# real-stanford/flingbot

Hardware: AMD Instinct MI355X
Metric: sim steps/sec (64x64-particle cloth) (higher is better)
Workload: dtype f32

## Files before the change

flingbot_amd/csrc/fs_fused_grid_kernel.h:

```cpp
#pragma once
#include "fs_fused_kernel.h"

#define FG_PLANE (FS_FUSED_MAX_PARTICLES * 4)
#define FG_PAD 1024
#define FG_OFF_XX FG_PAD
#define FG_OFF_X0 (FG_OFF_XX + 4 * FG_PLANE)
#define FG_OFF_CACC (FG_OFF_X0 + 3 * FG_PLANE)
#define FG_OFF_CUR (FG_OFF_CACC + FS_FUSED_CSET_CAP * 16)
#define FG_OFF_ITEMS (FG_OFF_CUR + FS_FUSED_CUR_BYTES)
#define FG_OFF_SCAN (FG_OFF_ITEMS + FS_FUSED_MAX_PARTICLES * 2)
#define FG_OFF_CSET (FG_OFF_SCAN + 64)
#define FG_OFF_CHIST (FG_OFF_CSET + FS_FUSED_CSET_CAP * 2)
#define FG_OFF_ROWL (FG_OFF_CHIST + 512)
#define FG_OFF_KZ (FG_OFF_ROWL + 1024)
#define FG_OFF_KS (FG_OFF_KZ + 1024)
#define FG_OFF_COLL (FG_OFF_KS + 1024)
#define FG_OFF_RCNT (FG_OFF_COLL + 512)
#define FG_LDS_BYTES (FG_OFF_RCNT + 512)
static_assert(FG_OFF_ROWL % 8 == 0 && (FG_OFF_KZ - FG_OFF_ROWL) % 8 == 0, "row tables are read as ds_read_b64 pairs");
static_assert((FG_OFF_COLL - FG_OFF_KS) % 256 == 0, "column tables share one address, rows as ds_read2st64_b32 offsets");
static_assert(FG_LDS_BYTES <= 160 * 1024, "grid-64 kernel: the LDS of one CU");
static_assert(FG_OFF_CACC % 16 == 0 && FG_OFF_CUR == FG_OFF_CACC + FS_FUSED_CSET_CAP * 16, "set and queue accumulators: one array");
#ifndef FG_SINGLES
#define FG_SINGLES 1
// ... 74 lines not shown
    unsigned short *items = (unsigned short *)(smem + FG_OFF_ITEMS);
    int *wave_tot = (int *)(smem + FG_OFF_SCAN);
    float *rowL = (float *)(smem + FG_OFF_ROWL);

#ifdef FS_BLOCK_CLOCKS
    const unsigned long long tc_start = __builtin_amdgcn_s_memtime(), tr_start = __builtin_amdgcn_s_memrealtime();
#endif
#ifdef FS_TIMING
    unsigned long long ts_acc[16] = {0, 0, 0, 0, 0, 0, 0, 0, 0, 0, 0, 0, 0, 0, 0, 0};
    unsigned long long ts_last = __builtin_amdgcn_s_memtime();
#endif
    const int e = ids[blockIdx.x];
    if (e < 0) return;
    const FsEnvDev &E = envs[e];
    const FsShapesDev &sh = shapes[e];
    const FsFusedConsts c = fs_fused_consts(E, sh);
    const int n = c.n;
    const unsigned un = (unsigned)n;
    const int t = threadIdx.x, lane = t & 63, w = t >> 6;
    const int dimz = n >> 6;

    FsVec4 *const g_pos = E.pos;
    const FsVec4 *const g_rest = E.rest;
    const fs_gci g_phase = (fs_gci)E.phase;
    const fs_gi g_nlist = (fs_gi)E.nlist, g_ncount = (fs_gi)E.ncount;
    const fs_gci g_ell_j = (fs_gci)E.ell_j;
    const fs_gcf g_ell_len = (fs_gcf)E.ell_len, g_ell_k = (fs_gcf)E.ell_k;
    const fs_gcf g_L = (fs_gcf)E.g64_L;
    const int max_deg = E.max_deg;
    const fs_gcu g_near = (fs_gcu)E.restnear_w;

    int find_mode = 0;
    {
        const int ph0 = g_phase[0];
        int differs = 0;
        for (int i = t; i < n; i += FS_FUSED_THREADS) differs |= (g_phase[i] != ph0);
        if (t == 0) wave_tot[0] = 0;
        __syncthreads();
        if (differs) atomicOr(&wave_tot[0], 1);
        __syncthreads();
        const int mixed = wave_tot[0];
        __syncthreads();
        if (!mixed) {
            if (!(ph0 & FS_PHASE_SELF_COLLIDE)) find_mode = 3;
            else if (!(ph0 & FS_PHASE_SELF_COLLIDE_FILTER)) find_mode = 2;
            else if (E.restnear_ok == 2 && FS_STENCIL_FILTER) find_mode = 4;
            else if (E.restnear_ok) find_mode = 1;
        }
    }
    for (int q = t; q < FG_OFF_X0 / 4; q += FS_FUSED_THREADS) ((float *)smem)[q] = 0.0f;
    __syncthreads();
    for (int i = t; i < n; i += FS_FUSED_THREADS) {
        const FsVec4 p = fs_ld4(g_pos, i);
        Xx[i] = p.x; Xy[i] = p.y; Xz[i] = p.z; Xw[i] = p.w;
        X0x[i] = p.x; X0y[i] = p.y; X0z[i] = p.z;
    }
    if (t < 256) {
        const int r = t & 63, s = 8 + (t >> 6);
        rowL[t] = r < dimz ? g_L[(unsigned)s * un + (unsigned)(r * 64 + 2)] : 0.0f;
    }
    constexpr int XS_DX[4] = {-1, -2, +1, +2};
    constexpr int SH_DX[4] = {+1, -1, -1, +1}, SH_DZ[4] = {-1, -1, +1, +1};
    constexpr int ZS_DZ[4] = {-1, -2, +1, +2};
    float *colL = (float *)(smem + FG_OFF_COLL);
    if (t < 128) {
        const int col = t & 63, q = t >> 6;
        const int dxq = q == 0 ? -1 : -2;
        colL[t] = (unsigned)(col + dxq) < 64u ? g_L[(unsigned)q * un + (unsigned)(2 * 64 + col)] : 0.0f;
    }
    float *rcnt = (float *)(smem + FG_OFF_RCNT);
    if (t < 128) rcnt[t] = t > 0 ? c.relax / (float)t : 0.0f;
    if (t < 256) {
        const int c64 = t & 63, q = t >> 6;
        const int sdx = (q == 0 || q == 3) ? +1 : -1, sslot = q < 2 ? 2 + q : 4 + q;
        const int zdz = q < 2 ? -1 - q : q - 1;
        ((float *)(smem + FG_OFF_KS))[t] = (unsigned)(c64 + sdx) < 64u ? E.g64_kh[sslot] : 0.0f;
        ((float *)(smem + FG_OFF_KZ))[t] = (c64 < dimz && (unsigned)(c64 + zdz) < (unsigned)dimz) ? E.g64_kh[8 + q] : 0.0f;
    }
    const float kh0 = E.g64_kh[0], kh1 = E.g64_kh[1];
    unsigned nvalid = 0u;
#pragma unroll
    for (int k = 0; k < FS_FUSED_PPT; ++k) {
        const int row = FG_ROW(w, k);
        int cnt = 0;
#pragma unroll
        for (int q = 0; q < 4; ++q) {
            cnt += ((unsigned)(lane + XS_DX[q]) < 64u) ? 1 : 0;
            cnt += ((unsigned)(lane + SH_DX[q]) < 64u && (unsigned)(row + SH_DZ[q]) < (unsigned)dimz) ? 1 : 0;
            cnt += ((unsigned)(row + ZS_DZ[q]) < (unsigned)dimz) ? 1 : 0;
        }
        nvalid |= (unsigned)cnt << (8 * k);
    }
    __syncthreads();
    unsigned fastmask = 0u;
    {
        constexpr int cdx[FS_G64_SLOTS] = FS_G64_DX_LIST, cdz[FS_G64_SLOTS] = FS_G64_DZ_LIST;
#pragma unroll
        for (int k = 0; k < FS_FUSED_PPT; ++k) {
            const int row = FG_ROW(w, k), i = row * 64 + lane;
            bool differs = false;
            if (i < n) {
                const float wi = Xw[i];
                differs = !(wi > 0.0f);
#pragma unroll
                for (int q = 0; q < FS_G64_SLOTS; ++q) {
                    const bool in = (unsigned)(lane + cdx[q]) < 64u && (unsigned)(row + cdz[q]) < (unsigned)dimz;
                    if (in) differs |= Xw[i + cdz[q] * 64 + cdx[q]] != wi;
                }
            }
            if (i < n && __builtin_amdgcn_ballot_w64(differs) == 0ull) fastmask |= 1u << k;
        }
        fastmask = (unsigned)__builtin_amdgcn_readfirstlane((int)fastmask);
    }

    FsVec4 sx[FS_FUSED_PPT], sv[FS_FUSED_PPT];
#pragma unroll
    for (int k = 0; k < FS_FUSED_PPT; ++k) {
        const int i = t + k * FS_FUSED_THREADS;
        sx[k] = FsVec4{0.0f, 0.0f, 0.0f, 0.0f};
        sv[k] = FsVec4{0.0f, 0.0f, 0.0f, 0.0f};
        if (i < n) {
            sv[k] = fs_ld4o(E.vel, (unsigned)i);
            sx[k] = FsVec4{X0x[i], X0y[i], X0z[i], Xw[i]};
        }
    }

    FS_TS(0)
#pragma unroll 1
    for (int frame = 0; frame < n_steps; ++frame) {
#pragma unroll 1
        for (int sub = 0; sub < c.substeps; ++sub) {
            FsVec4 xp[FS_FUSED_PPT];
            {
                unsigned tl = (unsigned)t;
                asm volatile("" : "+v"(tl));
                for (unsigned q = tl; q < FS_FUSED_BUCKETS / 2; q += FS_FUSED_THREADS) ((unsigned *)cursor)[q] = 0u;
                FsFusedConsts cf = c;
                asm volatile("" : "+v"(cf.h), "+v"(cf.g0), "+v"(cf.g1), "+v"(cf.g2), "+v"(cf.damping));
#pragma unroll
                for (int k = 0; k < FS_FUSED_PPT; ++k) {
                    const unsigned i = tl + (unsigned)(k * FS_FUSED_THREADS);
                    xp[k] = FsVec4{0.0f, 0.0f, 0.0f, 0.0f};
                    if (i < un) xp[k] = fs_fused_predict(cf, sx[k], sv[k]);
                }
#pragma unroll
                for (int k = 0; k < FS_FUSED_PPT; ++k) {
                    const unsigned i = tl + (unsigned)(k * FS_FUSED_THREADS);
                    if (i < un) fs_st4o(E.x0, i, sx[k]);
                }
            }
            FS_TS(12)
            __syncthreads();
            const fs_lu fill = (fs_lu)(smem + FG_OFF_XX + 2 * FG_PLANE);
            if (find_mode == 4) {
                unsigned tl = (unsigned)t;
                asm volatile("" : "+v"(tl));
                for (unsigned q = tl; q < FS_FUSED_MAX_PARTICLES; q += FS_FUSED_THREADS) fill[q] = 0u;
            }
            unsigned xslot[2];
            {
                int slot_of[FS_FUSED_PPT] = {0, 0, 0, 0};
                fs_fused_build_grid(c, xp, cursor, items, wave_tot, X0x, X0y, X0z, slot_of);
                xslot[0] = (unsigned)slot_of[0] | ((unsigned)slot_of[1] << 16);
                xslot[1] = (unsigned)slot_of[2] | ((unsigned)slot_of[3] << 16);
            }
            FS_TS(1)
            const FsFindConsts fc = {n, c.ncap, c.rad2, c.inv_rad, find_mode, E.gp_dimx, E.gp_magic};
            if (find_mode == 4) {
                int *const any_over = wave_tot;
                if (t == 0) *any_over = 0;
                int sb0 = 0, sb1 = 0, sb2 = 0, sb3 = 0;
#pragma unroll 1
                for (int k = 0; k < FS_FUSED_PPT; ++k) {
                    const int qs = t + k * FS_FUSED_THREADS;
                    if (qs >= n) break;
                    const int i = items[qs];
                    const FsVec4 xi = FsVec4{X0x[qs], X0y[qs], X0z[qs], 0.0f};
                    const int shape_bits = (int)(fs_shape_candidates(E.p, sh, sub, xi.x, xi.y, xi.z) << FS_SHAPE_MASK_SHIFT);
                    if (k == 0) sb0 = shape_bits; else if (k == 1) sb1 = shape_bits; else if (k == 2) sb2 = shape_bits; else sb3 = shape_bits;
                    fs_pair_find_neighbors(fc, i, qs, xi, (fs_lcus)cursor, (fs_lcus)items, g_nlist, (fs_lus)(smem + FG_OFF_XX) + t,
                                           (fs_lcf)X0x, fill);
                }
                FS_TS(2)
                __syncthreads();
                FS_TS(3)
                unsigned overmask = 0u;
#pragma unroll 1
                for (int k = 0; k < FS_FUSED_PPT; ++k) {
                    const int qs = t + k * FS_FUSED_THREADS;
                    if (qs >= n) break;
                    const int i = items[qs];
                    const int cnt = (int)fill[i];
                    const int shape_bits = k == 0 ? sb0 : k == 1 ? sb1 : k == 2 ? sb2 : sb3;
                    if (cnt > c.ncap) {
                        overmask |= 1u << k;
                        continue;
                    }
                    fs_pair_sort_column(n, i, cnt, g_nlist);
                    g_ncount[i] = cnt | shape_bits;
                }
                if (overmask) atomicOr(any_over, 1);
                __syncthreads();
                if (*any_over) {
                    FsNearWords none;
#pragma unroll
                    for (int q = 0; q < 8; ++q) none.w[q] = 0xffffffffu;
#pragma unroll 1
                    for (int k = 0; k < FS_FUSED_PPT; ++k) {
                        if (!((overmask >> k) & 1u)) continue;
                        const int qs = t + k * FS_FUSED_THREADS;
                        const int i = items[qs];
                        const FsVec4 xi = FsVec4{X0x[qs], X0y[qs], X0z[qs], 0.0f};
                        const int shape_bits = k == 0 ? sb0 : k == 1 ? sb1 : k == 2 ? sb2 : sb3;
                        g_ncount[i] = fs_fused_find_neighbors<true>(fc, i, xi, (fs_lcus)cursor, (fs_lcus)items, g_phase, g_rest, g_nlist,
                                                                    none, (fs_lus)(smem + FG_OFF_XX) + t, (fs_lcf)X0x) | shape_bits;
                    }
                    __syncthreads();
                }
                FS_TS(15)
            } else {
#pragma unroll 1
                for (int qs = t; qs < n; qs += FS_FUSED_THREADS) {
                    const int i = items[qs];
                    const FsVec4 xi = FsVec4{X0x[qs], X0y[qs], X0z[qs], 0.0f};
                    const int shape_bits = (int)(fs_shape_candidates(E.p, sh, sub, xi.x, xi.y, xi.z) << FS_SHAPE_MASK_SHIFT);
                    FsNearWords near;
#pragma unroll
                    for (int q = 0; q < 8; ++q) near.w[q] = find_mode == 1 ? g_near[(unsigned)q * un + (unsigned)i] : 0xffffffffu;
                    g_ncount[i] = (find_mode == 3 ? 0
                                                  : fs_fused_find_neighbors<false>(fc, i, xi, (fs_lcus)cursor, (fs_lcus)items, g_phase,
                                                                                   g_rest, g_nlist, near,
                                                                                   (fs_lus)(smem + FG_OFF_XX) + t, (fs_lcf)X0x)) |
                                  shape_bits;
                }
                FS_TS(2)
                __syncthreads();
                FS_TS(3)
            }
            FsVec4 p0r[FS_FUSED_PPT];
            int cword[FS_FUSED_PPT];
            {
                unsigned tl = (unsigned)t;
                asm volatile("" : "+v"(tl));
#pragma unroll
                for (int k = 0; k < FS_FUSED_PPT; ++k) {
                    const unsigned i = tl + (unsigned)(k * FS_FUSED_THREADS);
                    p0r[k] = fs_ld4o(E.x0, i < un ? i : 0u);
                }
                const unsigned wl = tl >> 6, ll = tl & 63u;
#pragma unroll
                for (int k = 0; k < FS_FUSED_PPT; ++k) {
                    const unsigned i = (unsigned)FG_ROW(wl, k) * 64u + ll;
                    cword[k] = fs_ldo((const int *)E.ncount, i < un ? i : 0u);
                }
#pragma unroll
                for (int k = 0; k < FS_FUSED_PPT; ++k) {
                    const unsigned i = tl + (unsigned)(k * FS_FUSED_THREADS);
                    const unsigned s = (xslot[k >> 1] >> (16 * (k & 1))) & 0xffffu;
                    const float x = X0x[s], y = X0y[s], z = X0z[s];
                    if (i < un) {
                        Xx[i] = x; Xy[i] = y; Xz[i] = z; Xw[i] = p0r[k].w;
                    } else {
                        Xx[i] = 0.0f; Xy[i] = 0.0f; Xz[i] = 0.0f; Xw[i] = 0.0f;
                    }
                }
            }

            FS_TS(13)
            unsigned short *cset = (unsigned short *)(smem + FG_OFF_CSET);
            FsVec4 *cacc = (FsVec4 *)(smem + FG_OFF_CACC);
            int *chist = (int *)(smem + FG_OFF_CHIST);
            if (t < 128) chist[t] = 0;
            int *nsingles = (int *)(smem + FG_OFF_SCAN);
            if (t == 0) *nsingles = 0;
            __syncthreads();
            {
                unsigned tl = (unsigned)t;
                asm volatile("" : "+v"(tl));
#pragma unroll
                for (int k = 0; k < FS_FUSED_PPT; ++k) {
                    const unsigned i = tl + (unsigned)(k * FS_FUSED_THREADS);
                    if (i < un) { X0x[i] = p0r[k].x; X0y[i] = p0r[k].y; X0z[i] = p0r[k].z; }
                }
            }
            unsigned tq = (unsigned)t;
            asm volatile("" : "+v"(tq));
            const int wq = (int)(tq >> 6), lq = (int)(tq & 63u);
            int ccls[FS_FUSED_PPT];
#pragma unroll
            for (int k = 0; k < FS_FUSED_PPT; ++k) {
                const int i = FG_ROW(wq, k) * 64 + lq;
                int cc = 0;
                if (i < n && Xw[i] > 0.0f) cc = cword[k] & FS_NCOUNT_MASK;
                ccls[k] = cc > 96 ? 96 : cc;
                if (ccls[k] > 0) atomicAdd(&chist[ccls[k]], 1);
            }
            __syncthreads();
            fs_fused_count_offsets(chist, t);
            __syncthreads();
            FsVec4 *squeue = cacc + FS_FUSED_CSET_CAP;
            unsigned slotw[2] = {~0u, ~0u};
#pragma unroll
            for (int k = 0; k < FS_FUSED_PPT; ++k) {
                if (ccls[k] > 0) {
                    const int i = FG_ROW(wq, k) * 64 + lq;
                    unsigned slot = FG_SLOT_INLINE;
                    const int pos = atomicAdd(&chist[ccls[k]], 1);
                    if (pos < FS_FUSED_CSET_CAP) {
                        cset[pos] = (unsigned short)i;
                        slot = (unsigned)pos;
                    }
#if FG_SINGLES
                    else if (ccls[k] <= 16) {
                        const int sp = atomicAdd(nsingles, 1);
                        if (sp < FG_SINGLES_CAP) {
                            slot = (unsigned)(FS_FUSED_CSET_CAP + sp);
                            squeue[sp].w = __int_as_float(i | (fs_ldo((const int *)E.nlist, (unsigned)i) << 12) | ((ccls[k] - 1) << 28));
                        }
                    }
#endif
                    slotw[k >> 1] = (slotw[k >> 1] & ~(0xffffu << (16 * (k & 1)))) | (slot << (16 * (k & 1)));
                }
            }
            FS_TS(14)
            __syncthreads();
            const int csize = chist[0] < FS_FUSED_CSET_CAP ? chist[0] : FS_FUSED_CSET_CAP;
            const int n_singles = *nsingles < FG_SINGLES_CAP ? *nsingles : FG_SINGLES_CAP;
            const int i2 = t < csize ? (int)cset[t] : -1;
            int cnt2 = 0, cj2[FS_FUSED_PREFETCH_CAND];
#pragma unroll
            for (int q = 0; q < FS_FUSED_PREFETCH_CAND; ++q) cj2[q] = 0;
            if (i2 >= 0) {
                cnt2 = g_ncount[i2] & FS_NCOUNT_MASK;
#pragma unroll
                for (int q = 0; q < FS_FUSED_PREFETCH_CAND; ++q) cj2[q] = g_nlist[(unsigned)q * un + (unsigned)i2];
            }
            static_assert(FG_SINGLES_CAP <= 2 * FG_SINGLES_LANES, "two queue entries per lane");
            unsigned qw0 = 0u, qw1 = 0u;
#if FG_SINGLES
            if (t >= 64 && t - 64 < n_singles) qw0 = (unsigned)__float_as_int(squeue[t - 64].w);
            if (t >= 64 && t - 64 + FG_SINGLES_LANES < n_singles) qw1 = (unsigned)__float_as_int(squeue[t - 64 + FG_SINGLES_LANES].w);
            __syncthreads();
#endif

            FS_TS(4)
#pragma unroll 1
            for (int it = 0; it < c.iters; ++it) {
                unsigned cpack = 0u;
                float rold[2][3], rnew[2][3];
#pragma unroll
                for (int q = 0; q < 6; ++q) { rold[q / 3][q % 3] = 0.0f; rnew[q / 3][q % 3] = 0.0f; }
// ... 382 lines not shown
```

flingbot_amd/csrc/fs_fused_kernel.h:

```cpp
#pragma once
#include "fs_constraints.h"
#include "fs_pair_search.h"

#ifndef FS_FUSED_THREADS
#define FS_FUSED_THREADS 1024
#endif
#define FS_FUSED_PPT (4096 / FS_FUSED_THREADS)
#define FS_FUSED_MAX_PARTICLES (FS_FUSED_THREADS * FS_FUSED_PPT)
#define FS_FUSED_MAX_DEG 64
#ifndef FS_STENCIL_FILTER
#define FS_STENCIL_FILTER 1
#endif
#ifndef FS_FUSED_BUCKET_BITS
#define FS_FUSED_BUCKET_BITS 13
#endif
#define FS_FUSED_BUCKETS (1 << FS_FUSED_BUCKET_BITS)
#define FS_FUSED_CUR_BYTES (FS_FUSED_BUCKETS * 2)
#define FS_FUSED_SLOTS 16

#define FS_FUSED_OFF_DICT 0
#define FS_FUSED_OFF_X (FS_FUSED_OFF_DICT + 256 * 8)
#define FS_FUSED_OFF_X0 (FS_FUSED_OFF_X + FS_FUSED_MAX_PARTICLES * 16)
#define FS_FUSED_OFF_CUR (FS_FUSED_OFF_X0 + FS_FUSED_MAX_PARTICLES * 12)
#define FS_FUSED_OFF_ITEMS (FS_FUSED_OFF_CUR + FS_FUSED_CUR_BYTES)
// ... 247 lines not shown
template <bool STENCIL = false, int ST = FS_NB_STAGED_STREAM>
__device__ __forceinline__ void fs_fused_accept(const FsFindConsts &c, int i, int j, FsNbListT<ST> &L, int &phi, FsVec4 &ri,
                                                bool &have_meta, fs_gci phase, const FsVec4 *rest, fs_gi nlist,
                                                const FsNearWords &near) {
    if (STENCIL) {
        const int rj = (int)__umulhi((unsigned)j, c.magic), ri_ = (int)__umulhi((unsigned)i, c.magic);
        const int cj = j - rj * c.dimx, ci = i - ri_ * c.dimx;
        if ((unsigned)(rj - ri_ + 1) <= 2u && (unsigned)(cj - ci + 1) <= 2u) return;
    } else if (c.mode == 0) {
        if (!have_meta) {
            phi = phase[i];
            ri = fs_ld4(rest, i);
            have_meta = true;
        }
        const FsVec4 rj = fs_ld4(rest, j);
        if (!fs_pair_allowed(phi, phase[j], ri, rj, c.rad2)) return;
    } else if (c.mode == 4) {
        const int rj = (int)__umulhi((unsigned)j, c.magic), ri_ = (int)__umulhi((unsigned)i, c.magic);
        const int cj = j - rj * c.dimx, ci = i - ri_ * c.dimx;
        if ((unsigned)(rj - ri_ + 1) <= 2u && (unsigned)(cj - ci + 1) <= 2u) return;
    } else if (c.mode == 1) {
        const uint32_t jj = (uint32_t)j | ((uint32_t)j << 16);
        uint32_t hit = 0u;
#pragma unroll
        for (int q = 0; q < 8; ++q) {
            const uint32_t x = near.w[q] ^ jj;
            hit |= (x - 0x00010001u) & ~x & 0x80008000u;
        }
        if (hit) return;
    }
    bool dup = false;
#pragma unroll
    for (int q = 0; q < ST; ++q) dup |= (j == L.a[q]);
    if (dup) return;
    FS_CNT_LANE(4, 1)
    const int gcap = c.ncap - ST;
    if (j > L.a[ST - 1]) {
        fs_fused_global_insert<ST>(c.n, i, j, gcap, L.gcnt, nlist);
        return;
    }
    int t = j;
#pragma unroll
    for (int q = 0; q < ST; ++q) {
        const int lo = min(L.a[q], t);
        t = max(L.a[q], t);
        L.a[q] = lo;
    }
    if (t != FS_NB_EMPTY) fs_fused_global_insert<ST>(c.n, i, t, gcap, L.gcnt, nlist);
}

template <int ST>
__device__ __forceinline__ int fs_fused_nb_finish(const FsFindConsts &c, int i, const FsNbListT<ST> &L, fs_gi nlist) {
    int st = 0;
    const size_t n = (size_t)c.n;
#pragma unroll
    for (int q = 0; q < ST; ++q) {
        if (L.a[q] != FS_NB_EMPTY) { nlist[(size_t)q * n + i] = L.a[q]; ++st; }
    }
    const int total = st + L.gcnt;
    return total < c.ncap ? total : c.ncap;
}

typedef __attribute__((address_space(3))) const int *fs_lci;
typedef __attribute__((address_space(3))) const float *fs_lcf;
typedef __attribute__((address_space(3))) const fs_f4 *fs_lcf4;
typedef __attribute__((address_space(3))) const unsigned short *fs_lcus;
typedef __attribute__((address_space(3))) unsigned short *fs_lus;

template <bool STENCIL = false>
__device__ __forceinline__ void fs_fused_drain(const FsFindConsts &c, int i, int &qn, FsNbListT<FS_NB_STAGED_FUSED> &L, int &phi, FsVec4 &ri,
                                               bool &have_meta, fs_lcus items, fs_lus queue, fs_gci phase,
                                               const FsVec4 *rest, fs_gi nlist, const FsNearWords &near) {
    int e = 0, qb = 0;
    unsigned m = 0u;
    for (;;) {
        if (!m) {
            if (e == qn) break;
            const unsigned u = queue[e * FS_FUSED_THREADS];
            ++e;
            m = u & 15u;
            qb = (int)(u >> 4) << 2;
        }
        FS_CNT_WAVE(5, 1)
        const int j = items[qb + __builtin_ctz(m)];
        m &= m - 1u;
        if (j == i) continue;
        FS_CNT_LANE(3, 1)
        fs_fused_accept<STENCIL, FS_NB_STAGED_FUSED>(c, i, j, L, phi, ri, have_meta, phase, rest, nlist, near);
    }
    qn = 0;
}

template <bool STENCIL = false>
__device__ __noinline__ int fs_fused_find_neighbors(const FsFindConsts c, int i, const FsVec4 xi, fs_lcus cursor,
                                                       fs_lcus items, fs_gci phase, const FsVec4 *rest, fs_gi nlist,
                                                       const FsNearWords near,
                                                       fs_lus queue , fs_lcf XSx) {
    fs_lcf XSy = XSx + FS_FUSED_MAX_PARTICLES, XSz = XSy + FS_FUSED_MAX_PARTICLES;
    const int cx = (int)floorf(xi.x * c.inv_rad), cy = (int)floorf(xi.y * c.inv_rad), cz = (int)floorf(xi.z * c.inv_rad);
    int phi = 0, qn = 0;
    FsNbListT<FS_NB_STAGED_FUSED> L = fs_nb_empty<FS_NB_STAGED_FUSED>();
    FsVec4 ri = FsVec4{0.0f, 0.0f, 0.0f, 0.0f};
    bool have_meta = false;
#ifdef FS_TIMING
    const unsigned long long tf0 = __builtin_amdgcn_s_memtime();
#endif
    for (int dz = -1; dz <= 1; ++dz)
        for (int dy = -1; dy <= 1; ++dy) {
            const int b0 = (fs_fused_row(cy + dy, cz + dz) + cx - 1) & (FS_FUSED_BUCKETS - 1);
            const int wrap = b0 + 2 - (FS_FUSED_BUCKETS - 1);
            for (int seg = 0; seg < 2; ++seg) {
                int beg, end;
                if (seg == 0) {
                    beg = (b0 == 0) ? 0 : (int)cursor[b0 - 1];
                    end = (int)cursor[wrap > 0 ? FS_FUSED_BUCKETS - 1 : b0 + 2];
                } else {
                    if (wrap <= 0) break;
                    beg = 0;
                    end = (int)cursor[wrap - 1];
                }
                FS_CNT_WAVE(0, 1)
                FS_CNT_LANE(2, end - beg)
                for (int q = beg & ~3; q < end; q += 4) {
                    FS_CNT_WAVE(1, 1)
                    const fs_f4 ax = *(fs_lcf4)(XSx + q), ay = *(fs_lcf4)(XSy + q), az = *(fs_lcf4)(XSz + q);
                    const fs_f4 ex = xi.x - ax, ey = xi.y - ay, ez = xi.z - az;
                    const fs_f4 d2 = ex * ex + ey * ey + ez * ez;
                    unsigned m = (unsigned)(d2.x < c.rad2) | ((unsigned)(d2.y < c.rad2) << 1) |
                                 ((unsigned)(d2.z < c.rad2) << 2) | ((unsigned)(d2.w < c.rad2) << 3);
                    const int lo = beg - q > 0 ? beg - q : 0, hi = end - q < 4 ? end - q : 4;
                    m &= ((1u << (hi - lo)) - 1u) << lo;
                    if (m) {
                        if (qn == FS_FUSED_FINDQ)
                            fs_fused_drain<STENCIL>(c, i, qn, L, phi, ri, have_meta, items, queue, phase, rest, nlist, near);
                        queue[qn * FS_FUSED_THREADS] = (unsigned short)(((unsigned)q << 2) | m);
                        ++qn;
                    }
                }
            }
        }
#ifdef FS_TIMING
    const unsigned long long tf1 = __builtin_amdgcn_s_memtime();
    FS_DBG_COUNT(6, tf1 - tf0)
#endif
    fs_fused_drain<STENCIL>(c, i, qn, L, phi, ri, have_meta, items, queue, phase, rest, nlist, near);
#ifdef FS_TIMING
    FS_DBG_COUNT(7, __builtin_amdgcn_s_memtime() - tf1)
#endif
    return fs_fused_nb_finish(c, i, L, nlist);
}

#define FS_PAIR_FINDQ 16
typedef __attribute__((address_space(3))) unsigned *fs_lu;

__device__ __forceinline__ void fs_pair_drain(const FsFindConsts &c, int i, int row_i, int col_i, int cx, int cy, int cz, int &qn,
                                              unsigned long long &tags, fs_lcus items, fs_lus queue, fs_lcf XSx, fs_lu fill,
                                              fs_gi nlist) {
    fs_lcf XSy = XSx + FS_FUSED_MAX_PARTICLES, XSz = XSy + FS_FUSED_MAX_PARTICLES;
    int e = 0, qb = 0, r = 0;
    unsigned m = 0u;
    for (;;) {
        if (!m) {
            if (e == qn) break;
            const unsigned u = queue[e * FS_FUSED_THREADS];
            r = (int)(tags >> (4 * e)) & 7;
            ++e;
            m = u & 15u;
            qb = (int)(u >> 4) << 2;
        }
        FS_CNT_WAVE(5, 1)
        const int s = qb + __builtin_ctz(m);
        m &= m - 1u;
        FS_CNT_LANE(3, 1)
        const int j = items[s];
        const int row_j = (int)__umulhi((unsigned)j, c.magic), col_j = j - row_j * c.dimx;
        if ((unsigned)(row_j - row_i + 1) <= 2u && (unsigned)(col_j - col_i + 1) <= 2u) continue;
        const int ddx = (int)floorf(XSx[s] * c.inv_rad) - cx, ddy = (int)floorf(XSy[s] * c.inv_rad) - cy,
                  ddz = (int)floorf(XSz[s] * c.inv_rad) - cz;
        if (!fs_pair_run_takes(r, ddx, ddy, ddz)) continue;
        FS_CNT_LANE(4, 1)
        const unsigned ki = __hip_atomic_fetch_add(fill + i, 1u, __ATOMIC_RELAXED, __HIP_MEMORY_SCOPE_WORKGROUP);
        if (ki < (unsigned)c.ncap) nlist[ki * (unsigned)c.n + (unsigned)i] = j;
        const unsigned kj = __hip_atomic_fetch_add(fill + j, 1u, __ATOMIC_RELAXED, __HIP_MEMORY_SCOPE_WORKGROUP);
        if (kj < (unsigned)c.ncap) nlist[kj * (unsigned)c.n + (unsigned)j] = i;
    }
    qn = 0;
    tags = 0ull;
}

__device__ __noinline__ void fs_pair_find_neighbors(const FsFindConsts c, int i, int qs, const FsVec4 xi, fs_lcus cursor,
                                                    fs_lcus items, fs_gi nlist, fs_lus queue ,
                                                    fs_lcf XSx, fs_lu fill) {
    fs_lcf XSy = XSx + FS_FUSED_MAX_PARTICLES, XSz = XSy + FS_FUSED_MAX_PARTICLES;
    const int cx = (int)floorf(xi.x * c.inv_rad), cy = (int)floorf(xi.y * c.inv_rad), cz = (int)floorf(xi.z * c.inv_rad);
    const int row_i = (int)__umulhi((unsigned)i, c.magic), col_i = i - row_i * c.dimx;
    int qn = 0;
    unsigned long long tags = 0ull;
#ifdef FS_TIMING
    const unsigned long long tf0 = __builtin_amdgcn_s_memtime();
#endif
    for (int r = 0; r < FS_PAIR_RUNS; ++r)
        for (int seg = 0; seg < 2; ++seg) {
            int beg, end;
            if (!fs_pair_run_segment(cursor, FS_FUSED_BUCKET_BITS, r, seg, qs, cx, cy, cz, beg, end)) break;
            FS_CNT_WAVE(0, 1)
            FS_CNT_LANE(2, end - beg)
            for (int q = beg & ~3; q < end; q += 4) {
                FS_CNT_WAVE(1, 1)
                const fs_f4 ax = *(fs_lcf4)(XSx + q), ay = *(fs_lcf4)(XSy + q), az = *(fs_lcf4)(XSz + q);
                const fs_f4 ex = xi.x - ax, ey = xi.y - ay, ez = xi.z - az;
                const fs_f4 d2 = ex * ex + ey * ey + ez * ez;
                unsigned m = (unsigned)(d2.x < c.rad2) | ((unsigned)(d2.y < c.rad2) << 1) |
                             ((unsigned)(d2.z < c.rad2) << 2) | ((unsigned)(d2.w < c.rad2) << 3);
                const int lo = beg - q > 0 ? beg - q : 0, hi = end - q < 4 ? end - q : 4;
                m &= ((1u << (hi - lo)) - 1u) << lo;
                if (m) {
                    if (qn == FS_PAIR_FINDQ)
                        fs_pair_drain(c, i, row_i, col_i, cx, cy, cz, qn, tags, items, queue, XSx, fill, nlist);
                    queue[qn * FS_FUSED_THREADS] = (unsigned short)(((unsigned)q << 2) | m);
                    tags |= (unsigned long long)r << (4 * qn);
                    ++qn;
                }
            }
        }
#ifdef FS_TIMING
    const unsigned long long tf1 = __builtin_amdgcn_s_memtime();
    FS_DBG_COUNT(6, tf1 - tf0)
#endif
    fs_pair_drain(c, i, row_i, col_i, cx, cy, cz, qn, tags, items, queue, XSx, fill, nlist);
#ifdef FS_TIMING
    FS_DBG_COUNT(7, __builtin_amdgcn_s_memtime() - tf1)
#endif
}

__device__ __forceinline__ void fs_pair_sort_column(int n, int i, int cnt, fs_gi nlist) {
    if (cnt < 2) return;
    const fs_gi col = nlist + i;
    const unsigned un = (unsigned)n;
    if (cnt <= 4) {
        int a0 = col[0], a1 = col[un], a2 = cnt > 2 ? col[2u * un] : FS_NB_EMPTY, a3 = cnt > 3 ? col[3u * un] : FS_NB_EMPTY;
        int lo, hi;
        lo = min(a0, a1); hi = max(a0, a1); a0 = lo; a1 = hi;
        lo = min(a2, a3); hi = max(a2, a3); a2 = lo; a3 = hi;
        lo = min(a0, a2); hi = max(a0, a2); a0 = lo; a2 = hi;
        lo = min(a1, a3); hi = max(a1, a3); a1 = lo; a3 = hi;
        lo = min(a1, a2); hi = max(a1, a2); a1 = lo; a2 = hi;
        col[0] = a0; col[un] = a1;
        if (cnt > 2) col[2u * un] = a2;
        if (cnt > 3) col[3u * un] = a3;
        return;
    }
    for (int a = 1; a < cnt; ++a) {
        const int v = col[(unsigned)a * un];
        int b = a;
        while (b > 0) {
            const int p = col[(unsigned)(b - 1) * un];
            if (p <= v) break;
            col[(unsigned)b * un] = p;
            --b;
        }
        col[(unsigned)b * un] = v;
    }
}


__device__ __forceinline__ void fs_fused_count_offsets(int *chist, int t) {
    if (t >= 64) return;
    const int h0 = chist[2 * t], h1 = chist[2 * t + 1];
    const int pair = h0 + h1;
    int inc = pair;
    for (int off = 1; off < 64; off <<= 1) {
        const int o = __shfl_down(inc, off, 64);
        if (t + off < 64) inc += o;
    }
    const int above = inc - pair;
    chist[2 * t + 1] = above;
    chist[2 * t] = above + h1;
}

__device__ __forceinline__ void fs_fused_shape_contacts(FsAcc &a, const FsFusedConsts &c, const FsParams &p,
                                                        const FsShapesDev &sh, int sub, unsigned mask, float xi0, float xi1,
                                                        float xi2, float ri0, float ri1, float ri2) {
    if (c.n_planes == 1) {
        if (mask & 1u) fs_plane_contact(a, xi0, xi1, xi2, ri0, ri1, ri2, c.pl0, c.pl1, c.pl2, c.pl3, c.cd, c.mu_s, c.mu_k);
    } else {
        for (int q = 0; q < c.n_planes; ++q)
            if ((mask >> q) & 1u)
                fs_plane_contact(a, xi0, xi1, xi2, ri0, ri1, ri2, p.planes[q][0], p.planes[q][1], p.planes[q][2],
                                 p.planes[q][3], c.cd, c.mu_s, c.mu_k);
    }
    if (c.n_shapes == 0 || __builtin_amdgcn_ballot_w64((mask >> FS_SHAPE_SPHERE_BIT) != 0u) == 0ull) return;
    const float S = (float)c.substeps;
    for (int q = 0; q < c.n_shapes; ++q)
        if ((mask >> (FS_SHAPE_SPHERE_BIT + q)) & 1u) {
            float c0, c1, c2, s0, s1, s2;
            fs_shape_sweep(sh, q, sub, S, c0, c1, c2, s0, s1, s2);
            fs_sphere_contact(a, xi0, xi1, xi2, ri0, ri1, ri2, c0, c1, c2, sh.pos[q].w, s0, s1, s2, c.cd, c.mu_s, c.mu_k);
        }
}

template <int SLOTS, bool FAST>
__device__ __forceinline__ void fs_fused_spring_block(FsAcc &a, const char *smem, const uint32_t (&jw)[SLOTS / 2 > 0 ? SLOTS / 2 : 1],
                                                      const uint32_t (&cw)[SLOTS / 2 > 0 ? SLOTS / 2 : 1], float xi0, float xi1,
                                                      float xi2, float wi, float kscale) {
    FsVec4 xj = *(const FsVec4 *)(smem + FS_FUSED_OFF_X + (jw[0] & 0xffffu));
    float2 lk = *(const float2 *)(smem + FS_FUSED_OFF_DICT + (cw[0] & 0xffffu));
#pragma unroll
    for (int s = 0; s < SLOTS; ++s) {
        FsVec4 xj_next = xj;
        float2 lk_next = lk;
        if (s + 1 < SLOTS) {
            const uint32_t joff = (jw[(s + 1) >> 1] >> (16 * ((s + 1) & 1))) & 0xffffu;
            const uint32_t coff = (cw[(s + 1) >> 1] >> (16 * ((s + 1) & 1))) & 0xffffu;
            xj_next = *(const FsVec4 *)(smem + FS_FUSED_OFF_X + joff);
            lk_next = *(const float2 *)(smem + FS_FUSED_OFF_DICT + coff);
        }
        if (FAST) fs_spring_fast(a, xi0, xi1, xi2, xj, lk.x, lk.y);
        else fs_spring_bf(a, xi0, xi1, xi2, wi, xj, lk.x, lk.y * kscale);
        __builtin_amdgcn_sched_barrier(0);
        xj = xj_next;
        lk = lk_next;
    }
}

#if FS_FUSED_PPT <= 4
#define FS_SLOTWORD(sp, k) ((sp)[0])
#else
#define FS_SLOTWORD(sp, k) (((k) >> 2) ? (sp)[1] : (sp)[0])
#endif

template <int SLOTS>
__global__ __launch_bounds__(FS_FUSED_THREADS) void fs_k_fused_step(const FsEnvDev *__restrict__ envs, const FsShapesDev *__restrict__ shapes,
                                                                    const int *ids, int n_steps) {
    constexpr bool COMPACT = SLOTS > 0;
    constexpr int JW = COMPACT ? SLOTS / 2 : 1;
    extern __shared__ __attribute__((aligned(16))) char smem[];
    FsVec4 *X = (FsVec4 *)(smem + FS_FUSED_OFF_X);
    float *X0x = (float *)(smem + FS_FUSED_OFF_X0);
    float *X0y = X0x + FS_FUSED_MAX_PARTICLES;
    float *X0z = X0y + FS_FUSED_MAX_PARTICLES;
    unsigned short *cursor = (unsigned short *)(smem + FS_FUSED_OFF_CUR);
    unsigned short *items = (unsigned short *)(smem + FS_FUSED_OFF_ITEMS);
    int *wave_tot = (int *)(smem + FS_FUSED_OFF_SCAN);

#ifdef FS_TIMING
    unsigned long long ts_acc[12] = {0, 0, 0, 0, 0, 0, 0, 0, 0, 0, 0, 0};
    unsigned long long ts_last = __builtin_amdgcn_s_memtime();
#define FS_TS(k)                                                     \
    {                                                                \
        const unsigned long long now = __builtin_amdgcn_s_memtime(); \
        ts_acc[k] += now - ts_last;                                  \
        ts_last = now;                                               \
    }
#else
#define FS_TS(k)
#endif
    const int e = ids[blockIdx.x];
    if (e < 0) return;
    const FsEnvDev &E = envs[e];
    const FsShapesDev &sh = shapes[e];
    const FsFusedConsts c = fs_fused_consts(E, sh);
    const int n = c.n;
    const int kmax = (n + FS_FUSED_THREADS - 1) / FS_FUSED_THREADS;
    const unsigned un = (unsigned)n;
    const int t = threadIdx.x;

    FsVec4 *const g_pos = E.pos, *const g_vel = E.vel;
    const FsVec4 *const g_rest = E.rest;
    const fs_gci g_phase = (fs_gci)E.phase;
    const fs_gi g_nlist = (fs_gi)E.nlist, g_ncount = (fs_gi)E.ncount;
    const fs_gci g_ell_j = (fs_gci)E.ell_j;
    const fs_gcf g_ell_len = (fs_gcf)E.ell_len, g_ell_k = (fs_gcf)E.ell_k;
    const fs_gcu g_nbr = (fs_gcu)E.nbr_w, g_code = (fs_gcu)E.code_w;
    const int max_deg = E.max_deg;

    float2 dict_e = make_float2(0.0f, 0.0f);
    bool dict_bad = false;
    if (COMPACT && t < 256) {
        const fs_gcf g_dict = (fs_gcf)E.dict;
        dict_e = make_float2(g_dict[2 * t], g_dict[2 * t + 1]);
        dict_bad = t < E.dict_size && (dict_e.y < 0.0f || (dict_e.y * 0.5f) * 2.0f != dict_e.y);
    }
    const fs_gcu g_near = (fs_gcu)E.restnear_w;
    int find_mode = 0;
    bool dict_halved = false;
    {
        const int ph0 = g_phase[0];
        int differs = 0;
        for (int i = t; i < n; i += FS_FUSED_THREADS) differs |= (g_phase[i] != ph0);
        if (t == 0) { wave_tot[0] = 0; wave_tot[1] = 0; }
        __syncthreads();
        if (differs) atomicOr(&wave_tot[0], 1);
        if (dict_bad) atomicOr(&wave_tot[1], 1);
        __syncthreads();
        const int mixed = wave_tot[0];
        dict_halved = COMPACT && wave_tot[1] == 0;
        __syncthreads();
        if (!mixed) {
            if (!(ph0 & FS_PHASE_SELF_COLLIDE)) find_mode = 3;
            else if (!(ph0 & FS_PHASE_SELF_COLLIDE_FILTER)) find_mode = 2;
            else if (E.restnear_ok == 2 && FS_STENCIL_FILTER) find_mode = 4;
            else if (E.restnear_ok) find_mode = 1;
        }
    }
// ... 354 lines not shown
```

flingbot_amd/csrc/fs_pair_search.h:

```cpp
#pragma once

#define FS_PAIR_RUNS 5
#define FS_PAIR_OWN_RUN 4

__host__ __device__ inline int fs_pair_row(int cy, int cz, int bits) {
    const unsigned h = (unsigned)cy * 0x85EBCA77u + (unsigned)cz * 0xC2B2AE3Du;
    return (int)((h ^ (h >> 15)) * 0x2C1B3C6Du >> (32 - bits));
}

__host__ __device__ inline void fs_pair_run_row(int r, int &dy, int &dz) {
    dz = r < 3 ? 1 : 0;
    dy = r < 3 ? r - 1 : (r == 3 ? 1 : 0);
}

template <typename Cursor>
__host__ __device__ inline bool fs_pair_run_segment(const Cursor cursor, int bits, int r, int seg, int qs, int cx, int cy, int cz,
                                                    int &beg, int &end) {
    const int nb = 1 << bits;
    int dy, dz;
    fs_pair_run_row(r, dy, dz);
    const bool own = r == FS_PAIR_OWN_RUN;
    const int b0 = (fs_pair_row(cy + dy, cz + dz, bits) + cx - (own ? 0 : 1)) & (nb - 1);
    const int wrap = b0 + (own ? 1 : 2) - (nb - 1);
    if (seg == 0) {
        beg = own ? qs + 1 : (b0 == 0 ? 0 : (int)cursor[b0 - 1]);
        end = (int)cursor[wrap > 0 ? nb - 1 : b0 + (own ? 1 : 2)];
        return true;
    }
    if (wrap <= 0) return false;
    beg = 0;
    end = (int)cursor[wrap - 1];
    return true;
}

__host__ __device__ inline bool fs_pair_run_takes(int r, int ddx, int ddy, int ddz) {
    int dy, dz;
    fs_pair_run_row(r, dy, dz);
    if (ddy != dy || ddz != dz) return false;
    return r == FS_PAIR_OWN_RUN ? (unsigned)ddx <= 1u : (unsigned)(ddx + 1) <= 2u;
}

__host__ __device__ inline bool fs_pair_owns(int ddx, int ddy, int ddz, int slot_i, int slot_j) {
    if ((unsigned)(ddx + 1) > 2u || (unsigned)(ddy + 1) > 2u || (unsigned)(ddz + 1) > 2u) return false;
    if (ddz != 0) return ddz > 0;
    if (ddy != 0) return ddy > 0;
    if (ddx != 0) return ddx > 0;
    return slot_j > slot_i;
}
```

Baseline: 147,700.

## Keep first four neighbour ids in LDS and sort columns with a 16-wide network

```diff
diff --git a/flingbot_amd/csrc/fs_fused_grid_kernel.h b/flingbot_amd/csrc/fs_fused_grid_kernel.h
--- a/flingbot_amd/csrc/fs_fused_grid_kernel.h
+++ b/flingbot_amd/csrc/fs_fused_grid_kernel.h
@@ -250,6 +250,10 @@
             FS_TS(12)
             __syncthreads();
             const fs_lu fill = (fs_lu)(smem + FG_OFF_XX + 2 * FG_PLANE);
+            const fs_lus heads = (fs_lus)(smem + FG_OFF_XX + 3 * FG_PLANE);
+            static_assert(FG_OFF_CACC - (FG_OFF_XX + 3 * FG_PLANE) == FS_PAIR_HEADS_HI * 2, "heads: rows 2, 3 start at the set's accumulators");
+            static_assert(FS_FUSED_CSET_CAP * 16 >= 2 * FS_FUSED_MAX_PARTICLES * 2 && FG_PLANE >= 2 * FS_FUSED_MAX_PARTICLES * 2,
+                          "heads: two rows of 16-bit ids per region");
             if (find_mode == 4) {
                 unsigned tl = (unsigned)t;
                 asm volatile("" : "+v"(tl));
@@ -277,7 +281,7 @@
                     const int shape_bits = (int)(fs_shape_candidates(E.p, sh, sub, xi.x, xi.y, xi.z) << FS_SHAPE_MASK_SHIFT);
                     if (k == 0) sb0 = shape_bits; else if (k == 1) sb1 = shape_bits; else if (k == 2) sb2 = shape_bits; else sb3 = shape_bits;
                     fs_pair_find_neighbors(fc, i, qs, xi, (fs_lcus)cursor, (fs_lcus)items, g_nlist, (fs_lus)(smem + FG_OFF_XX) + t,
-                                           (fs_lcf)X0x, fill);
+                                           (fs_lcf)X0x, fill, heads);
                 }
                 FS_TS(2)
                 __syncthreads();
@@ -294,7 +298,7 @@
                         overmask |= 1u << k;
                         continue;
                     }
-                    fs_pair_sort_column(n, i, cnt, g_nlist);
+                    fs_pair_sort_column(n, i, cnt, g_nlist, (fs_lcus)heads);
                     g_ncount[i] = cnt | shape_bits;
                 }
                 if (overmask) atomicOr(any_over, 1);
diff --git a/flingbot_amd/csrc/fs_fused_kernel.h b/flingbot_amd/csrc/fs_fused_kernel.h
--- a/flingbot_amd/csrc/fs_fused_kernel.h
+++ b/flingbot_amd/csrc/fs_fused_kernel.h
@@ -423,10 +423,19 @@
 
 #define FS_PAIR_FINDQ 16
 typedef __attribute__((address_space(3))) unsigned *fs_lu;
+#define FS_PAIR_HEADS_HI (4 * FS_FUSED_MAX_PARTICLES * 4 / 2)
+#define FS_PAIR_HEAD(heads, k, p) (heads)[((k) & 1) * FS_FUSED_MAX_PARTICLES + ((k) >> 1) * FS_PAIR_HEADS_HI + (p)]
+static_assert(FS_PAIR_HEADS == 4, "two rows of heads per LDS region");
+
+__device__ __forceinline__ void fs_pair_append(int ncap, unsigned un, unsigned p, int q, fs_lu fill, fs_lus heads, fs_gi nlist) {
+    const unsigned k = __hip_atomic_fetch_add(fill + p, 1u, __ATOMIC_RELAXED, __HIP_MEMORY_SCOPE_WORKGROUP);
+    if (k < (unsigned)FS_PAIR_HEADS) FS_PAIR_HEAD(heads, k, p) = (unsigned short)q;
+    else if (k < (unsigned)ncap) nlist[k * un + p] = q;
+}
 
 __device__ __forceinline__ void fs_pair_drain(const FsFindConsts &c, int i, int row_i, int col_i, int cx, int cy, int cz, int &qn,
                                               unsigned long long &tags, fs_lcus items, fs_lus queue, fs_lcf XSx, fs_lu fill,
-                                              fs_gi nlist) {
+                                              fs_lus heads, fs_gi nlist) {
     fs_lcf XSy = XSx + FS_FUSED_MAX_PARTICLES, XSz = XSy + FS_FUSED_MAX_PARTICLES;
     int e = 0, qb = 0, r = 0;
     unsigned m = 0u;
@@ -450,10 +459,8 @@
                   ddz = (int)floorf(XSz[s] * c.inv_rad) - cz;
         if (!fs_pair_run_takes(r, ddx, ddy, ddz)) continue;
         FS_CNT_LANE(4, 1)
-        const unsigned ki = __hip_atomic_fetch_add(fill + i, 1u, __ATOMIC_RELAXED, __HIP_MEMORY_SCOPE_WORKGROUP);
-        if (ki < (unsigned)c.ncap) nlist[ki * (unsigned)c.n + (unsigned)i] = j;
-        const unsigned kj = __hip_atomic_fetch_add(fill + j, 1u, __ATOMIC_RELAXED, __HIP_MEMORY_SCOPE_WORKGROUP);
-        if (kj < (unsigned)c.ncap) nlist[kj * (unsigned)c.n + (unsigned)j] = i;
+        fs_pair_append(c.ncap, (unsigned)c.n, (unsigned)i, j, fill, heads, nlist);
+        fs_pair_append(c.ncap, (unsigned)c.n, (unsigned)j, i, fill, heads, nlist);
     }
     qn = 0;
     tags = 0ull;
@@ -461,7 +468,7 @@
 
 __device__ __noinline__ void fs_pair_find_neighbors(const FsFindConsts c, int i, int qs, const FsVec4 xi, fs_lcus cursor,
                                                     fs_lcus items, fs_gi nlist, fs_lus queue ,
-                                                    fs_lcf XSx, fs_lu fill) {
+                                                    fs_lcf XSx, fs_lu fill, fs_lus heads) {
     fs_lcf XSy = XSx + FS_FUSED_MAX_PARTICLES, XSz = XSy + FS_FUSED_MAX_PARTICLES;
     const int cx = (int)floorf(xi.x * c.inv_rad), cy = (int)floorf(xi.y * c.inv_rad), cz = (int)floorf(xi.z * c.inv_rad);
     const int row_i = (int)__umulhi((unsigned)i, c.magic), col_i = i - row_i * c.dimx;
@@ -487,7 +494,7 @@
                 m &= ((1u << (hi - lo)) - 1u) << lo;
                 if (m) {
                     if (qn == FS_PAIR_FINDQ)
-                        fs_pair_drain(c, i, row_i, col_i, cx, cy, cz, qn, tags, items, queue, XSx, fill, nlist);
+                        fs_pair_drain(c, i, row_i, col_i, cx, cy, cz, qn, tags, items, queue, XSx, fill, heads, nlist);
                     queue[qn * FS_FUSED_THREADS] = (unsigned short)(((unsigned)q << 2) | m);
                     tags |= (unsigned long long)r << (4 * qn);
                     ++qn;
@@ -498,29 +505,50 @@
     const unsigned long long tf1 = __builtin_amdgcn_s_memtime();
     FS_DBG_COUNT(6, tf1 - tf0)
 #endif
-    fs_pair_drain(c, i, row_i, col_i, cx, cy, cz, qn, tags, items, queue, XSx, fill, nlist);
+    fs_pair_drain(c, i, row_i, col_i, cx, cy, cz, qn, tags, items, queue, XSx, fill, heads, nlist);
 #ifdef FS_TIMING
     FS_DBG_COUNT(7, __builtin_amdgcn_s_memtime() - tf1)
 #endif
 }
 
-__device__ __forceinline__ void fs_pair_sort_column(int n, int i, int cnt, fs_gi nlist) {
-    if (cnt < 2) return;
+__device__ __forceinline__ void fs_pair_sort_column(int n, int i, int cnt, fs_gi nlist, fs_lcus heads) {
+    if (cnt < 1) return;
     const fs_gi col = nlist + i;
     const unsigned un = (unsigned)n;
+    int a0 = (int)FS_PAIR_HEAD(heads, 0, i), a1 = (int)FS_PAIR_HEAD(heads, 1, i), a2 = (int)FS_PAIR_HEAD(heads, 2, i),
+        a3 = (int)FS_PAIR_HEAD(heads, 3, i);
+    if (cnt < 2) a1 = FS_NB_EMPTY;
+    if (cnt < 3) a2 = FS_NB_EMPTY;
+    if (cnt < 4) a3 = FS_NB_EMPTY;
     if (cnt <= 4) {
-        int a0 = col[0], a1 = col[un], a2 = cnt > 2 ? col[2u * un] : FS_NB_EMPTY, a3 = cnt > 3 ? col[3u * un] : FS_NB_EMPTY;
         int lo, hi;
         lo = min(a0, a1); hi = max(a0, a1); a0 = lo; a1 = hi;
         lo = min(a2, a3); hi = max(a2, a3); a2 = lo; a3 = hi;
         lo = min(a0, a2); hi = max(a0, a2); a0 = lo; a2 = hi;
         lo = min(a1, a3); hi = max(a1, a3); a1 = lo; a3 = hi;
         lo = min(a1, a2); hi = max(a1, a2); a1 = lo; a2 = hi;
-        col[0] = a0; col[un] = a1;
+        col[0] = a0;
+        if (cnt > 1) col[un] = a1;
         if (cnt > 2) col[2u * un] = a2;
         if (cnt > 3) col[3u * un] = a3;
         return;
     }
+    if (cnt <= FS_PAIR_SORT_BOUND) {
+        int v[FS_PAIR_SORT_BOUND];
+        const unsigned last = (unsigned)(cnt - 1);
+        v[0] = a0; v[1] = a1; v[2] = a2; v[3] = a3;
+#pragma unroll
+        for (int a = FS_PAIR_HEADS; a < FS_PAIR_SORT_BOUND; ++a) v[a] = col[min((unsigned)a, last) * un];
+#pragma unroll
+        for (int a = FS_PAIR_HEADS + 1; a < FS_PAIR_SORT_BOUND; ++a)
+            if (a >= cnt) v[a] = FS_NB_EMPTY;
+        fs_pair_sort16(v);
+#pragma unroll
+        for (int a = 0; a < FS_PAIR_SORT_BOUND; ++a)
+            if (a < cnt) col[(unsigned)a * un] = v[a];
+        return;
+    }
+    col[0] = a0; col[un] = a1; col[2u * un] = a2; col[3u * un] = a3;
     for (int a = 1; a < cnt; ++a) {
         const int v = col[(unsigned)a * un];
         int b = a;
diff --git a/flingbot_amd/csrc/fs_pair_search.h b/flingbot_amd/csrc/fs_pair_search.h
--- a/flingbot_amd/csrc/fs_pair_search.h
+++ b/flingbot_amd/csrc/fs_pair_search.h
@@ -47,3 +47,22 @@
     if (ddx != 0) return ddx > 0;
     return slot_j > slot_i;
 }
+
+#define FS_PAIR_HEADS 4
+#define FS_PAIR_SORT_BOUND 16
+#define FS_PAIR_SORT16_STEPS 63
+
+__host__ __device__ inline void fs_pair_sort16(int (&v)[FS_PAIR_SORT_BOUND]) {
+    constexpr unsigned char A[FS_PAIR_SORT16_STEPS] = {0, 2, 4, 6, 8, 10, 12, 14, 0, 1, 4, 5, 8, 9, 12, 13, 1, 5, 9, 13, 0,
+                                                       1, 2, 3, 8, 9, 10, 11, 2, 3, 10, 11, 1, 3, 5, 9, 11, 13, 0, 1, 2, 3,
+                                                       4, 5, 6, 7, 4, 5, 6, 7, 2, 3, 6, 7, 10, 11, 1, 3, 5, 7, 9, 11, 13};
+    constexpr unsigned char B[FS_PAIR_SORT16_STEPS] = {1, 3, 5, 7, 9, 11, 13, 15, 2, 3, 6, 7, 10, 11, 14, 15, 2, 6, 10, 14, 4,
+                                                       5, 6, 7, 12, 13, 14, 15, 4, 5, 12, 13, 2, 4, 6, 10, 12, 14, 8, 9, 10, 11,
+                                                       12, 13, 14, 15, 8, 9, 10, 11, 4, 5, 8, 9, 12, 13, 2, 4, 6, 8, 10, 12, 14};
+#pragma unroll
+    for (int q = 0; q < FS_PAIR_SORT16_STEPS; ++q) {
+        const int lo = v[A[q]] < v[B[q]] ? v[A[q]] : v[B[q]], hi = v[A[q]] < v[B[q]] ? v[B[q]] : v[A[q]];
+        v[A[q]] = lo;
+        v[B[q]] = hi;
+    }
+}
```

Result: faster. 154,600 (median of 6 runs) (+4.7%).
